# krisbrud/gym-auv

Hardware: AMD Instinct MI355X
Metric: env-steps/sec (higher is better)
Workload: dtype f64; 1 GPU; 4096 envs x 180 sensors per GPU, 50 static polygon obstacles (BASELINE configs[2]); envs_per_gpu=4096, n_sensors=180, total_envs=4096, parallelism=env-shard x1 (no step-path collective), ranks=1, hipgraph_steps=0, steps_per_launch=64, sub_batches=1, api=multi, step_mode=one_launch, roofline_step_mode=one_launch, actions=uniform, worlds_per_env=2, collective_backend=none, episodes_finished=212

## Files before the change

### gym_auv_amd/csrc/k1_dynamics.hip

```cpp
#include <hip/hip_ext.h>

#include "auv_device.h"

namespace {

struct Vec6 {
  double v[6];
};

#define AUV_DIVC(x, c) auv_div_const((x), (c), 1.0 / (c))
__device__ __forceinline__ double auv_div_const(double x, double c, double rc) {
  const double q = x * rc;
  const double r = fma(-q, c, x);
  return fma(r, rc, q);
}

struct Heading0 {
  double psi, s, c;
};

__device__ __forceinline__ Heading0 heading0(double psi) {
  Heading0 h;
  h.psi = psi;
  sincos(auv_princip(psi), &h.s, &h.c);
  return h;
}

__device__ __forceinline__ void stage_sincos(const Heading0& h0, const double psi, double* s, double* c) {
  const double dl = psi - h0.psi;
  if (fabs(dl) <= 0.125) {
    const double z = dl * dl;
    double ps = fma(z, 1.0 / 6227020800.0, -1.0 / 39916800.0);
    ps = fma(z, ps, 1.0 / 362880.0), ps = fma(z, ps, -1.0 / 5040.0), ps = fma(z, ps, 1.0 / 120.0);
    ps = fma(z, ps, -1.0 / 6.0);
    const double sd = fma(dl * z, ps, dl);
    double pc = fma(z, -1.0 / 87178291200.0, 1.0 / 479001600.0);
    pc = fma(z, pc, -1.0 / 3628800.0), pc = fma(z, pc, 1.0 / 40320.0), pc = fma(z, pc, -1.0 / 720.0);
    pc = fma(z, pc, 1.0 / 24.0), pc = fma(z, pc, -0.5);
    const double cd = fma(z, pc, 1.0);
    *s = fma(h0.s, cd, h0.c * sd);
    *c = fma(h0.c, cd, -(h0.s * sd));
  } else {
    sincos(auv_princip(psi), s, c);
  }
}

__device__ __forceinline__ Vec6 state_dot(const Vec6& y, double tau_u, double tau_r, const Heading0& h0) {
  const double m = 23.8, x_g = 0.046, I_z = 1.760, X_udot = -2.0, Y_vdot = -10.0, Y_rdot = 0.0,
               N_rdot = -1.0, N_vdot = 0.0, X_u = -2.0, Y_v = -7.0, Y_r = -0.1, N_v = -0.1, N_r = -0.5;
  const double m11 = m - X_udot, m22 = m - Y_vdot, m23 = m * x_g - Y_rdot, m32 = m * x_g - N_vdot,
               m33 = I_z - N_rdot;
  const double det = m22 * m33 - m23 * m32;
  const double i11 = 1.0 / m11, i22 = m33 / det, i23 = -m23 / det, i32 = -m32 / det, i33 = m22 / det;
  double s, c;
  stage_sincos(h0, y.v[2], &s, &c);
  double u = y.v[3], v = y.v[4], r = y.v[5];
  Vec6 o;
  o.v[0] = c * u + -s * v;
  o.v[1] = s * u + c * v;
  o.v[2] = r;
  double d0 = 2.0 * u;
  double d1 = 7.0 * v + -2.5425 * r;
  double d2 = -2.5425 * v + 1.422 * r;
  double n0 = -X_u * u;
  double n1 = -Y_v * v + (m * u - Y_r) * r;
  double n2 = -N_v * v + (m * x_g * u - N_r) * r;
  double r0 = tau_u - d0 - n0, r1 = 0.0 - d1 - n1, r2 = tau_r - d2 - n2;
  o.v[3] = i11 * r0;
  o.v[4] = i22 * r1 + i23 * r2;
  o.v[5] = i32 * r1 + i33 * r2;
  return o;
}

__device__ __forceinline__ void k1_action(const AuvDev& d, const void* __restrict__ actions, const int e, double* a0, double* a1, const int slot = -1) {
  size_t i = 2 * (size_t)e;
  if (slot >= 0) i += (size_t)slot * 2 * (size_t)d.n;
  else if (d.ring_slots > 1)
    i += (size_t)(d.ring_slot_host >= 0 ? d.ring_slot_host : *d.ring_pos) * 2 * (size_t)d.n;
  if (d.act_f64) {
    const double2 a = *(const double2*)((const double*)actions + i);
    *a0 = a.x, *a1 = a.y;
  } else {
    const float2 a = *(const float2*)((const float*)actions + i);
    *a0 = (double)a.x, *a1 = (double)a.y;
  }
}

__device__ __forceinline__ EnvPre k1_env(const AuvDev& d, const int e, const void* __restrict__ actions, const bool store) {
  const size_t n = (size_t)d.n;
  double a0, a1;
  k1_action(d, actions, e, &a0, &a1);
  if (isnan(a0) || isnan(a1)) a0 = a1 = 0.0;
  const double tu = auv_clip(a0, 0.0, 1.0) * d.cfg.thrust_max;
  const double tr = auv_clip(a1, -1.0, 1.0) * d.cfg.moment_max;
  const double h = d.cfg.dt;
  Vec6 y, t;
#pragma unroll
  for (int i = 0; i < 6; i++) y.v[i] = d.state[i * n + e];

  const Heading0 h0 = heading0(y.v[2]);
  Vec6 s1 = state_dot(y, tu, tr, h0);
#pragma unroll
  for (int i = 0; i < 6; i++) t.v[i] = y.v[i] + h * s1.v[i] / 4.0;
  Vec6 s2 = state_dot(t, tu, tr, h0);
#pragma unroll
  for (int i = 0; i < 6; i++) t.v[i] = y.v[i] + 3.0 * h * s1.v[i] / 32.0 + 9.0 * h * s2.v[i] / 32.0;
  Vec6 s3 = state_dot(t, tu, tr, h0);
#pragma unroll
  for (int i = 0; i < 6; i++)
    t.v[i] = y.v[i] + AUV_DIVC(1932.0 * h * s1.v[i], 2197.0) - AUV_DIVC(7200.0 * h * s2.v[i], 2197.0) +
             AUV_DIVC(7296.0 * h * s3.v[i], 2197.0);
  Vec6 s4 = state_dot(t, tu, tr, h0);
#pragma unroll
  for (int i = 0; i < 6; i++)
    t.v[i] = y.v[i] + AUV_DIVC(439.0 * h * s1.v[i], 216.0) - 8.0 * h * s2.v[i] + AUV_DIVC(3680.0 * h * s3.v[i], 513.0) -
             AUV_DIVC(845.0 * h * s4.v[i], 4104.0);
  Vec6 s5 = state_dot(t, tu, tr, h0);
#pragma unroll
  for (int i = 0; i < 6; i++)
    t.v[i] = y.v[i] - AUV_DIVC(8.0 * h * s1.v[i], 27.0) + 2 * h * s2.v[i] - AUV_DIVC(3544.0 * h * s3.v[i], 2565.0) +
             AUV_DIVC(1859.0 * h * s4.v[i], 4104.0) - AUV_DIVC(11.0 * h * s5.v[i], 40.0);
  Vec6 s6 = state_dot(t, tu, tr, h0);
#pragma unroll
  for (int i = 0; i < 6; i++)
    t.v[i] = y.v[i] + h * (AUV_DIVC(16.0 * s1.v[i], 135.0) + AUV_DIVC(6656.0 * s3.v[i], 12825.0) +
                           AUV_DIVC(28561.0 * s4.v[i], 56430.0) - AUV_DIVC(9.0 * s5.v[i], 50.0) + AUV_DIVC(2.0 * s6.v[i], 55.0));
  t.v[2] = auv_princip(t.v[2]);
  EnvPre pre;
  pre.cnt = d.counters[e];
  pre.cnt.y += 1;
#pragma unroll
  for (int i = 0; i < 6; i++) pre.s[i] = t.v[i];
  if (store) {
#pragma unroll
    for (int i = 0; i < 6; i++) d.state[i * n + e] = t.v[i];
    d.counters[e].y = pre.cnt.y;
  }
  return pre;
}

#define K1_GROUP 8
template <int K> __device__ __forceinline__ int k1_group_bcast32(const int x) {
  static_assert(K >= 0 && K < 8, "lane of the group");
  constexpr int q = K % 4, qp = q | (q << 2) | (q << 4) | (q << 6);
  const int a = __builtin_amdgcn_update_dpp(0, x, qp, 0xF, 0xF, true);
  return K < 4 ? __builtin_amdgcn_update_dpp(a, a, 0x114, 0xF, 0xA, false) : __builtin_amdgcn_update_dpp(a, a, 0x104, 0xF, 0x5, false);
}
template <int K> __device__ __forceinline__ double k1_group_bcast(const double t) {
  return __hiloint2double(k1_group_bcast32<K>(__double2hiint(t)), k1_group_bcast32<K>(__double2loint(t)));
}
__device__ __forceinline__ double k1_group(const AuvDev& d, const void* __restrict__ actions, const int e, const int lane,
                                           const double* y_in = nullptr, const int slot = -1, const double2* a_in = nullptr) {
  const int c = lane % K1_GROUP, gbase = lane - c;
  const size_t n = (size_t)d.n;
  const bool own = c < 6;
  double a0, a1;
  if (a_in) a0 = a_in->x, a1 = a_in->y;
  else k1_action(d, actions, e, &a0, &a1, slot);
  if (isnan(a0) || isnan(a1)) a0 = a1 = 0.0;
  const double tu = auv_clip(a0, 0.0, 1.0) * d.cfg.thrust_max;
  const double tr = auv_clip(a1, -1.0, 1.0) * d.cfg.moment_max;
  const double h = d.cfg.dt;
  const double y = y_in ? *y_in : d.state[(size_t)(own ? c : 0) * n + e];
  (void)gbase;
  const Heading0 h0 = heading0(k1_group_bcast<2>(y));
  auto sdot = [&](double t) {
    Vec6 v;
    v.v[0] = 0.0, v.v[1] = 0.0;
    v.v[2] = k1_group_bcast<2>(t), v.v[3] = k1_group_bcast<3>(t);
    v.v[4] = k1_group_bcast<4>(t), v.v[5] = k1_group_bcast<5>(t);
    const Vec6 o = state_dot(v, tu, tr, h0);
    double r = o.v[0];
#pragma unroll
    for (int i = 1; i < 6; i++) r = (c == i) ? o.v[i] : r;
    return r;
  };
  const double s1 = sdot(y);
  double t = y + h * s1 / 4.0;
  const double s2 = sdot(t);
  t = y + 3.0 * h * s1 / 32.0 + 9.0 * h * s2 / 32.0;
  const double s3 = sdot(t);
  t = y + AUV_DIVC(1932.0 * h * s1, 2197.0) - AUV_DIVC(7200.0 * h * s2, 2197.0) + AUV_DIVC(7296.0 * h * s3, 2197.0);
  const double s4 = sdot(t);
  t = y + AUV_DIVC(439.0 * h * s1, 216.0) - 8.0 * h * s2 + AUV_DIVC(3680.0 * h * s3, 513.0) - AUV_DIVC(845.0 * h * s4, 4104.0);
  const double s5 = sdot(t);
  t = y - AUV_DIVC(8.0 * h * s1, 27.0) + 2 * h * s2 - AUV_DIVC(3544.0 * h * s3, 2565.0) + AUV_DIVC(1859.0 * h * s4, 4104.0) -
      AUV_DIVC(11.0 * h * s5, 40.0);
  const double s6 = sdot(t);
  t = y + h * (AUV_DIVC(16.0 * s1, 135.0) + AUV_DIVC(6656.0 * s3, 12825.0) + AUV_DIVC(28561.0 * s4, 56430.0) -
               AUV_DIVC(9.0 * s5, 50.0) + AUV_DIVC(2.0 * s6, 55.0));
  if (c == 2) t = auv_princip(t);
  return t;
}

#ifndef AUV_DEVICE_FUNCS_ONLY
__global__ void __launch_bounds__(AUV_BLOCK) k1_dynamics(AuvDev d, const void* __restrict__ actions) {
  const int tid = blockIdx.x * blockDim.x + threadIdx.x;
  const int lane = threadIdx.x % AUV_WAVE;
  const int c = lane % K1_GROUP;
  const size_t n = (size_t)d.n;
  const bool live = tid / K1_GROUP < d.ne;
  const int e = d.e0 + (live ? tid / K1_GROUP : d.ne - 1);
  const double t = k1_group(d, actions, e, lane);
  if (live && c < 6) d.state[(size_t)c * n + e] = t;
  if (live && c == 0) d.counters[e].y += 1;
}
#endif

}

#ifndef AUV_DEVICE_FUNCS_ONLY
void auv_launch_k1(const AuvDev& d0, const void* actions, int dtype, hipStream_t st, hipEvent_t ev0, hipEvent_t ev1) {
  AuvDev d = d0;
  d.act_f64 = dtype == AUV_F64;
  const int per_block = AUV_BLOCK / K1_GROUP;
  dim3 grid((d.ne + per_block - 1) / per_block), block(AUV_BLOCK);
  hipExtLaunchKernelGGL(k1_dynamics, grid, block, 0, st, ev0, ev1, 0, d, actions);
}
#endif
```

### gym_auv_amd/csrc/k2_lidar.hip

```cpp
#include "auv_device.h"

namespace {

#define K2_KIND_MASK 0xff
#define K2_PIP_FLAG 0x100
struct ObsLds {
  int kind;
  int seg_off;
  int nseg;
  int start;
  int count;
  int wind;
};

struct EnvHdr {
  double px, py;
  double cpsi, spsi;
  int n_act;
  int pad[3];
};

__device__ __forceinline__ unsigned long long d2u(double x) { return (unsigned long long)__double_as_longlong(x); }
__device__ __forceinline__ double u2d(unsigned long long x) { return __longlong_as_double((long long)x); }

__device__ __forceinline__ int wrap_ray(int i, int S) {
  if (i < 0) i += S;
  if (i < 0) i += S;
  if (i >= S) i -= S;
  return i;
}

struct MoverSegs {
  double c, s, x, y, wd;
  __device__ __forceinline__ void vertex(int k, double& vx, double& vy) const {
    const double bx = (k <= 1) ? -wd / 2 : (k == 3 ? 3.0 / 2 * wd : wd / 2);
    const double by = (k == 0 || k == 4) ? -wd / 2 : (k == 3 ? 0.0 : wd / 2);
    const double x0 = 5.0 * wd / 18.0;
    const double xo = x0 - x0 * c, yo = 0.0 - x0 * s;
    vx = (c * bx + -s * by + xo) + x;
    vy = (s * bx + c * by + yo) + y;
  }
  __device__ __forceinline__ double4 operator[](int i) const {
    double ax, ay, bx, by;
    vertex(i, ax, ay);
    vertex(i == 4 ? 0 : i + 1, bx, by);
    return make_double4(ax, ay, bx, by);
  }
};

#ifndef K2_SEG_CAP
#define K2_SEG_CAP 96
#endif
#define K2_SEG_CAP_MIN 32
#ifndef K2_HIT_S
#define K2_HIT_S 256
#endif
#ifndef K2_RAW_CAP
#define K2_RAW_CAP 192
#endif
#ifndef K2_ITEM_RAYS
#define K2_ITEM_RAYS 6
#endif

__host__ __device__ __forceinline__ size_t k2_slice_bytes(int S, int k_max, int m_max, int cap) {
  size_t b = sizeof(EnvHdr) + (size_t)m_max * 32 + (size_t)cap * 32 + (size_t)S * 16 + (size_t)m_max * 16 +
             (size_t)S * 8 + (size_t)m_max * 8 + (size_t)k_max * sizeof(ObsLds) + (size_t)cap * 4 +
             (size_t)k_max * 4 + (size_t)(k_max + 1) * 4 + (size_t)k_max * 4 + (size_t)cap * 2 +
             (size_t)(cap + 2) * 2;
  return (b + 15) & ~(size_t)15;
}
__host__ __device__ __forceinline__ size_t k2_slice_bytes(const AuvDev& d) { return k2_slice_bytes(d.cfg.n_sensors, d.k_max, d.m_max, d.seg_cap); }

struct Slice {
  EnvHdr* hdr;
  double4* mvrot;
  double4* stage;
  double2* rayv;
  double2* mvcull;
  unsigned long long* dbits;
  double* mvw;
  ObsLds* obs;
  short2* span;
  int* act;
  int* sbase;
  int* par;
  unsigned short* owner;
  unsigned short* ioff;
  int cap;
  int* hits;
  double* hitw;
};

__device__ __forceinline__ MoverSegs mover_segs(const double4 rot, const double wd) {
  MoverSegs ms;
  ms.c = rot.x, ms.s = rot.y, ms.x = rot.z, ms.y = rot.w, ms.wd = wd;
  return ms;
}

__device__ __forceinline__ Slice carve(unsigned char* p, int S, int k_max, int m_max, int cap) {
  Slice s;
  s.hdr = (EnvHdr*)p;
  s.mvrot = (double4*)(s.hdr + 1);
  s.stage = s.mvrot + m_max;
  s.rayv = (double2*)(s.stage + cap);
  s.mvcull = s.rayv + S;
  s.dbits = (unsigned long long*)(s.mvcull + m_max);
  s.mvw = (double*)(s.dbits + S);
  s.obs = (ObsLds*)(s.mvw + m_max);
  s.span = (short2*)(s.obs + k_max);
  s.act = (int*)(s.span + cap);
  s.sbase = s.act + k_max;
  s.par = s.sbase + k_max + 1;
  s.owner = (unsigned short*)(s.par + k_max);
  s.ioff = s.owner + cap;
  s.cap = cap;
  const size_t r1 = 32 * (size_t)(m_max + cap), r2 = (size_t)((unsigned char*)(s.ioff + cap + 2) - (unsigned char*)s.mvw);
  const size_t hb = ((size_t)4 * S + 7) & ~(size_t)7;
  s.hits = nullptr, s.hitw = nullptr;
  if (S <= K2_HIT_S && hb + (size_t)8 * S <= r1) s.hits = (int*)s.mvrot, s.hitw = (double*)((unsigned char*)s.mvrot + hb);
  else if (S <= K2_HIT_S && hb <= r1 && (size_t)8 * S <= r2) s.hits = (int*)s.mvrot, s.hitw = s.mvw;
  return s;
}
__device__ __forceinline__ Slice carve(unsigned char* p, const AuvDev& d) { return carve(p, d.cfg.n_sensors, d.k_max, d.m_max, d.seg_cap); }

__device__ __forceinline__ void test_pair(const double4 w, const double tn, const double2 r,
                                          unsigned long long* slot) {
  const double den = r.x * w.w - r.y * w.z;
  const double un = w.x * r.y - w.y * r.x;
  const bool neg = den < 0.0;
  const double dn = neg ? -den : den, t1 = neg ? -tn : tn, u1 = neg ? -un : un;
  const bool hit = (dn != 0.0) & (t1 >= 0.0) & (t1 <= dn) & (u1 >= 0.0) & (u1 <= dn);
  if (hit) atomicMin(slot, d2u(tn / den));
}

__device__ __forceinline__ void test_pair_signed(const double4 ws, const double ta, const double2 r, unsigned long long* slot) {
  const double dn = r.x * ws.w - r.y * ws.z;
  const double u1 = ws.x * r.y - ws.y * r.x;
  const bool hit = (dn > 0.0) & (ta <= dn) & (u1 >= 0.0) & (u1 <= dn);
  if (hit) atomicMin(slot, d2u(ta / dn));
}

template <typename SegPtr>
__device__ __forceinline__ void sweep_unstaged(const ObsLds& o, int tid, int nthr, int S, double px, double py,
                                               const double2* rayv, unsigned long long* dbits, SegPtr g) {
  const int total = o.count * o.nseg;
  for (int q = tid; q < total; q += nthr) {
    const int ro = q / o.nseg, si = q - ro * o.nseg;
    const int i = wrap_ray(o.start + ro, S);
    const double4 s = g[si];
    const double4 w = make_double4(s.x - px, s.y - py, s.z - s.x, s.w - s.y);
    test_pair(w, w.x * w.w - w.y * w.z, rayv[i], &dbits[i]);
  }
}

template <typename SegPtr>
__device__ __forceinline__ int inside_flag_wave(double px, double py, SegPtr g, int nseg, int lane) {
  int on_any = 0, cross = 0;
  for (int sb = 0; sb < nseg; sb += AUV_WAVE) {
    const int si = sb + lane;
    bool on = false, cr = false;
    if (si < nseg) {
      const double4 s = g[si];
      const double sx = s.z - s.x, sy = s.w - s.y, dxa = px - s.x, dya = py - s.y;
      const double len2 = sx * sx + sy * sy, dot = dxa * sx + dya * sy;
      if (len2 == 0.0 || dot <= 0.0) on = (dxa == 0.0 && dya == 0.0);
      else if (dot >= len2) on = (px == s.z && py == s.w);
      else on = ((s.y - py) * sx - (s.x - px) * sy) == 0.0;
      if ((s.y > py) != (s.w > py)) cr = px < s.x + (py - s.y) * (s.z - s.x) / (s.w - s.y);
    }
    on_any |= __any(on);
    cross += __popcll(__ballot(cr));
  }
  return (on_any ? 2 : 0) | (cross & 1);
}

__device__ __forceinline__ void k2_stage_beams(const AuvDev& d, const int lane, const Slice& L) {
  const int S = d.cfg.n_sensors;
  for (int i = lane; i < S; i += AUV_WAVE) L.rayv[i] = d.beam_cs[i];
}

__device__ __forceinline__ void k2_rays(const AuvDev& d, const int lane, const Slice& L, const bool staged = false) {
  const int S = d.cfg.n_sensors;
  const double R = d.cfg.sensor_range;
  const double px = L.hdr->px, py = L.hdr->py;
  double sin_psi, cos_psi;
  if (S <= 4 * AUV_WAVE) {
    double2 b[4];
    if (!staged) {
#pragma unroll
      for (int q = 0; q < 4; q++) {
        const int i = q * AUV_WAVE + lane;
        b[q] = d.beam_cs[i < S ? i : 0];
      }
    }
    cos_psi = L.hdr->cpsi, sin_psi = L.hdr->spsi;
#pragma unroll
    for (int q = 0; q < 4; q++) {
      if (q * AUV_WAVE >= S) break;
      const int i = q * AUV_WAVE + lane;
      if (i < S) {
        if (staged) b[q] = L.rayv[i];
        const double c = cos_psi * b[q].x - sin_psi * b[q].y, s = sin_psi * b[q].x + cos_psi * b[q].y;
        double ex = px + c * R, ey = py + s * R;
        L.rayv[i] = make_double2(ex - px, ey - py);
        L.dbits[i] = d2u(2.0);
      }
    }
  } else {
    cos_psi = L.hdr->cpsi, sin_psi = L.hdr->spsi;
    for (int i = lane; i < S; i += AUV_WAVE) {
      const double2 b = staged ? L.rayv[i] : d.beam_cs[i];
      const double c = cos_psi * b.x - sin_psi * b.y, s = sin_psi * b.x + cos_psi * b.y;
      double ex = px + c * R, ey = py + s * R;
      L.rayv[i] = make_double2(ex - px, ey - py);
      L.dbits[i] = d2u(2.0);
    }
  }
  auv_wave_lds_sync();
}

template <bool WT = false, bool LD = false>
__device__ __forceinline__ void k2_movers(const AuvDev& d, const int e, const int lane, const Slice& L, const EnvDesc& ed,
                                          const int advance_movers) {
  const long long m0 = ed.m0;
  const int M = ed.M;
  for (int m = lane; m < M; m += AUV_WAVE) {
    double4 st = auv_ld4<LD>(&d.mover[(size_t)e * d.m_max + m]);
    const double4 par_m = d.mv_param[m0 + m];
    if (advance_movers) {
      const double dt = d.cfg.dt;
      const long long voff = d.mv_vtab_off[m0 + m];
      const int vlen = d.mv_vtab_len[m0 + m];
      st.w += dt;
      int idx = (int)floor(st.w);
      if (idx >= (int)par_m.w - 1) {
        st.w = 0.0;
        idx = 0;
        st.x = par_m.y;
        st.y = par_m.z;
      }
      if (idx > vlen - 1) idx = vlen - 1;
      double2 v = d.mv_vtab[voff + idx];
      double dx = dt * v.x, dy = dt * v.y;
      st.z = atan2(dy, dx);
      st.x = st.x + dx;
      st.y = st.y + dy;
      auv_st<WT>(&d.mover[(size_t)e * d.m_max + m], st);
    }
    const double wd = par_m.x;
    double s, c;
    sincos(st.z, &s, &c);
    const double x0 = 5.0 * wd / 18.0, dxc = wd / 2.0 - x0;
    L.mvcull[m] = make_double2(st.x + x0 + c * dxc, st.y + s * dxc);
    if (fabs(c) < 2.5e-16) c = 0.0;
    if (fabs(s) < 2.5e-16) s = 0.0;
    L.mvrot[m] = make_double4(c, s, st.x, st.y);
    L.mvw[m] = wd;
  }
}

struct K2Pre {
  int4 meta;
  double cx, cy, rho;
  uint8_t near;
};
template <bool LD = false>
__device__ __forceinline__ K2Pre k2_prefetch(const AuvDev& d, const int e, const int lane, const EnvDesc& ed) {
  K2Pre p;
  p.meta = make_int4(0, 0, 0, 0), p.cx = p.cy = p.rho = 0.0, p.near = 0;
  if (lane < ed.K) {
    p.meta = d.obs_meta[ed.k0 + lane];
    p.cx = d.obs_cull[3 * (ed.k0 + lane)], p.cy = d.obs_cull[3 * (ed.k0 + lane) + 1], p.rho = d.obs_cull[3 * (ed.k0 + lane) + 2];
    p.near = auv_ld<LD>(&d.nearby[(size_t)e * d.k_max + lane]);
  }
  return p;
}

template <bool WT = false>
__device__ __forceinline__ int k2_front(const AuvDev& d, const int e, const int lane, const Slice& L, const int advance_movers,
                        const EnvPre* pre = nullptr, const int movers_done = 0,
                        const K2Pre* kp = nullptr, const bool beams_staged = false, int2* lim_defer = nullptr) {
  const int S = d.cfg.n_sensors;
  const size_t n = (size_t)d.n;
  const int4 cnt = pre ? pre->cnt : d.counters[e];
  const double px = pre ? pre->s[0] : d.state[0 * n + e], py = pre ? pre->s[1] : d.state[1 * n + e],
               psi = pre ? pre->s[2] : d.state[2 * n + e];
  const EnvDesc ed = (pre && pre->ed) ? *pre->ed : d.env_desc[e];
  {
    double sn, co;
    sincos(psi, &sn, &co);
    if (lane == 0) L.hdr->cpsi = co, L.hdr->spsi = sn;
  }
  const long long k0 = ed.k0;
  const int K = ed.K;
  const double R = d.cfg.sensor_range, W = d.cfg.vessel_width;
  const double dangle = d.derived[4], inv_dangle = d.derived[5];
  if (lane == 0) {
    L.hdr->px = px, L.hdr->py = py;
    L.hdr->n_act = 0;
  }

  if (!movers_done) k2_movers<WT>(d, e, lane, L, ed, advance_movers);
  if (!d.cfg.use_lidar) return 0;

  const bool refresh = (cnt.y % d.cfg.sensor_interval_load_obstacles) == 0;
  if (refresh) {
    for (int kb = 0; kb < K; kb += AUV_WAVE) {
      const int k = kb + lane;
      int4 meta = make_int4(0, 0, 0, 0);
      double dc = 0.0, rho = 0.0;
      int state = 0;
      if (k < K) {
        meta = d.obs_meta[k0 + k];
        double cx, cy;
        if (meta.x == AUV_OBS_MOVER) {
          const double2 c2 = L.mvcull[meta.w];
          cx = c2.x, cy = c2.y, rho = L.mvw[meta.w] * sqrt(5.0) / 2.0;
        } else {
          cx = d.obs_cull[3 * (k0 + k)], cy = d.obs_cull[3 * (k0 + k) + 1], rho = d.obs_cull[3 * (k0 + k) + 2];
        }
        dc = sqrt((px - cx) * (px - cx) + (py - cy) * (py - cy));
        state = (dc - rho - W >= R + 1e-9) ? 0 : ((dc + rho - W < R - 1e-9) ? 1 : 2);
      }
      unsigned long long pin = __ballot(state == 2 && meta.x != AUV_OBS_RING && dc <= rho * (1.0 + 1e-9) + 1e-9);
      while (pin) {
        const int src = __ffsll((long long)pin) - 1;
        pin &= pin - 1;
        const int kind = __shfl(meta.x, src, AUV_WAVE), soff = __shfl(meta.y, src, AUV_WAVE),
                  nseg = __shfl(meta.z, src, AUV_WAVE), mi = __shfl(meta.w, src, AUV_WAVE);
        const int in = (kind == AUV_OBS_MOVER) ? inside_flag_wave(px, py, mover_segs(L.mvrot[mi], L.mvw[mi]), nseg, lane)
                                               : inside_flag_wave(px, py, d.seg + soff, nseg, lane);
// ... 704 lines not shown
```

### gym_auv_amd/csrc/k_step_fused.hip

```cpp
#include <cstdlib>
#include <hip/hip_ext.h>

#define AUV_DEVICE_FUNCS_ONLY
#include "auv_multi_geom.h"
#include "k1_dynamics.hip"
#include "k2_lidar.hip"
#include "k3_nav_reward.hip"

#ifndef AUV_K23_MIN_WAVES
#define AUV_K23_MIN_WAVES 4
#endif

#ifdef AUV_TEST_HOOKS
#define AUV_HOOK_SKEW(d) ((d).pair_skew)
#define AUV_HOOK_FAULT(d) ((d).pair_fault)
#else
#define AUV_HOOK_SKEW(d) 0
#define AUV_HOOK_FAULT(d) 0
#endif

namespace {

#define PAIR_EMPTY AUV_PAIR_EMPTY
#define PAIR_COLLISION AUV_PAIR_COLLISION
// ... 248 lines not shown
    __hip_atomic_store(pair_word + e, PAIR_EMPTY, __ATOMIC_RELAXED, __HIP_MEMORY_SCOPE_AGENT);
    __hip_atomic_store(k1_pkt + 8 * (size_t)e + 7, 0ull, __ATOMIC_RELAXED, __HIP_MEMORY_SCOPE_AGENT);
    __hip_atomic_store(hd + 7, 0ull, __ATOMIC_RELAXED, __HIP_MEMORY_SCOPE_AGENT);
    RewardIn in;
    const int collision = word == PAIR_COLLISION;
    in.closeness_reward = collision ? 0.0 : __longlong_as_double((long long)word);
    in.path_reward = no.rew_path, in.reached = no.reached, in.goal = no.goal, in.progress = no.progress;
    in.u = no.u, in.v = no.v, in.yaw_rate = no.r;
    in.cum = cum_in;
    in.cte100 = no.cte100, in.cte_sum = cte_sum_in;
    st.info64[8 * (size_t)e] = collision;
    do_reset = reward_apply(st, e, collision, cnt, in, reward_out, done_out, false);
  }
  unsigned long long m = __ballot(do_reset);
  if (m) {
    while (m) {
      const int src = __ffsll((long long)m) - 1;
      m &= m - 1;
      const int er2 = auv_uniform(__shfl(e, src, AUV_WAVE));
      const int wr = auv_uniform(__shfl(w, src, AUV_WAVE)), ep = auv_uniform(__shfl(cnt.z, src, AUV_WAVE));
      const AuvDev* dp = dk.self;
      asm volatile("" : "+s"(dp));
      const AuvDev& dr = *(const AuvDev*)(const __attribute__((address_space(4))) AuvDev*)dp;
      restore_env(dr, er2, auv_next_world_wave(dr, wr, lane), lane, ep, obs_out);
    }
  }
#ifdef AUV_STAMPS
  if (live && c == 0) d.stamps[(size_t)e * 16 + 15] = wall_clock64();
#endif
}

__global__ void __launch_bounds__(AUV_WAVE, AUV_K23_MIN_WAVES) k_step_roles(AuvDev dk, const void* __restrict__ actions,
                                                                           float* __restrict__ obs_out,
                                                                           float* __restrict__ reward_out,
                                                                           uint8_t* __restrict__ done_out) {
  const AuvDev& d = dk;
  extern __shared__ __align__(16) unsigned char smem[];
  const int lane = threadIdx.x;
  const int ne = d.ne;
  const int nk = 8 * ((ne + 63) / 64);
  const int nb = 8 * ((ne + 7) / 8);
  const int b = (int)blockIdx.x;
  if (b < nk) {
    __builtin_amdgcn_s_setprio(3);
    const int g = lane / K1_GROUP, c = lane % K1_GROUP;
    const int er = 8 * (8 * (b / 8) + g) + (b % 8);
    const bool live = er < ne;
    const int eg = d.e0 + (live ? er : ne - 1);
    const int y = d.counters[eg].y + 1;
    const int aborted = auv_uniform(*d.abort_flag);
    double t = 0.0;
    if (!aborted) t = k1_group(d, actions, eg, lane);
    unsigned long long* pk = d.k1_pkt + 8 * (size_t)eg;
    const unsigned long long word = aborted ? (c == 6 ? (unsigned long long)ROLES_ABORT_COUNTER : 0ull)
                                            : (c < 6 ? (unsigned long long)__double_as_longlong(t) : (c == 6 ? (unsigned long long)(unsigned)y : 0ull));
    const unsigned long long mark = roles_mark(roles_group_xor(word));
    if (live && !(AUV_HOOK_FAULT(d) == 2 && eg == d.e0))
      __hip_atomic_store(pk + c, c < 7 ? word : mark, __ATOMIC_RELAXED, __HIP_MEMORY_SCOPE_AGENT);
    if (d.ring_slots > 1 && d.ring_slot_host == -1 && lane == 0) {
      const int old = __hip_atomic_fetch_add(d.k1_done, 1, __ATOMIC_RELAXED, __HIP_MEMORY_SCOPE_AGENT);
      if (old == nk - 1) {
        *d.ring_pos = (*d.ring_pos + 1) % d.ring_slots;
        __hip_atomic_store(d.k1_done, 0, __ATOMIC_RELAXED, __HIP_MEMORY_SCOPE_AGENT);
      }
    }
#ifdef AUV_STAMPS
    if (live && c == 0) d.stamps[(size_t)eg * 16 + 0] = wall_clock64();
#endif
    return;
  }
  EnvPre pre;
  EnvDesc ed;
  if (b < nk + nb) {
    if (b - nk >= ne) return;
    const int e = auv_uniform(d.e0 + b - nk);
#ifdef AUV_STAMPS
    if (lane == 0) d.stamps[(size_t)e * 16 + 3] = wall_clock64();
#endif
    if (auv_uniform(*d.abort_flag)) return;
    ed = d.env_desc[e];
    pre.cnt = d.counters[e];
    pre.ed = &ed;
    const Slice L = carve(smem, d);
    k2_movers<true>(d, e, lane, L, ed, 1);
    const K2Pre kp = k2_prefetch(d, e, lane, ed);
    k2_stage_beams(d, lane, L);
#ifdef AUV_STAMPS
    if (lane == 0) d.stamps[(size_t)e * 16 + 1] = wall_clock64();
#endif
    {
      const int ws = roles_wait_state(d, e, lane, pre);
      if (ws) {
        if (ws == 2 && ed.M > 0 && lane == 0) auv_st<true>(d.broken + e, (uint8_t)1);
        return;
      }
    }
#ifdef AUV_STAMPS
    if (lane == 0) d.stamps[(size_t)e * 16 + 2] = wall_clock64();
#endif
    int n_act = 0;
    int2 lim0 = make_int2(INT32_MIN, INT32_MIN);
    if (AUV_RUN_L(d, 1)) n_act = k2_front<true>(d, e, lane, L, 1, &pre, 1, &kp, true, &lim0);
#ifdef AUV_STAMPS
    if (lane == 0) d.stamps[(size_t)e * 16 + 8] = wall_clock64();
#endif
    if (AUV_RUN_L(d, 3)) k2_stage_and_pairs(d, L, lane, n_act, pre.s[2]);
#ifdef AUV_STAMPS
    if (lane == 0) d.stamps[(size_t)e * 16 + 11] = wall_clock64();
#endif
    double term = 0.0;
    const int collision = k2_back<true>(d, e, lane, L, n_act, obs_out, &term, &lim0);
#ifdef AUV_STAMPS
    if (lane == 0) d.stamps[(size_t)e * 16 + 4] = wall_clock64();
#endif
    pair_publish_lidar(d, e, lane, collision, term);
#ifdef AUV_STAMPS
    if (lane == 0) d.stamps[(size_t)e * 16 + 14] = wall_clock64();
#endif
  } else if (b < nk + 2 * nb + AUV_HOOK_SKEW(d)) {
    const int el = b - nk - nb - AUV_HOOK_SKEW(d);
    if (el < 0 || el >= ne) return;
    const int e = auv_uniform(d.e0 + el);
    ed = d.env_desc[e];
    pre.cnt = d.counters[e];
    pre.ed = &ed;
#ifdef AUV_STAMPS
    if (lane == 0) d.stamps[(size_t)e * 16 + 12] = wall_clock64();
#endif
    if (roles_wait_state(d, e, lane, pre)) return;
#ifdef AUV_STAMPS
    if (lane == 0) d.stamps[(size_t)e * 16 + 5] = wall_clock64();
#endif
    NavNear nr;
    nr.A = nr.B = make_double2(0.0, 0.0), nr.cum = 0.0;
    if (AUV_RUN_N(d, 1)) {
      int* list = (int*)smem;
      const NavSpec sp = nav_bounds(d, e, lane, list, pre.s[0], pre.s[1], &ed);
      if (AUV_RUN_N(d, 2)) nr = nav_nearest(d, e, lane, list, pre.s[0], pre.s[1], sp);
    }
    roles_publish_search(d, e, lane, nr);
#ifdef AUV_STAMPS
    if (lane == 0) d.stamps[(size_t)e * 16 + 6] = wall_clock64();
#endif
  } else {
    const int f = b - nk - 2 * nb - AUV_HOOK_SKEW(d);
    if (f < 0 || f >= nk) return;
    __builtin_amdgcn_s_setprio(2);
    roles_finish_wave(d, f, lane, obs_out, reward_out, done_out);
  }
}

#define CARRY_WORDS 24

#ifdef AUV_STAMPS_MULTI
#define MSTAMP(e, k) do { if (lane == 0) stamp[(size_t)(e) * 16 + (k)] = wall_clock64(); } while (0)
#define MSTAMP_IF(cond, e, k) do { if (cond) stamp[(size_t)(e) * 16 + (k)] = wall_clock64(); } while (0)
#define MSTAMP_PARAM , unsigned long long* stamp
#define MSTAMP_ARG , stamp
#else
#define MSTAMP(e, k) do { } while (0)
#define MSTAMP_IF(cond, e, k) do { } while (0)
#define MSTAMP_PARAM
#define MSTAMP_ARG
#endif

__device__ __forceinline__ unsigned long long carry_ed_word(const EnvDesc& ed, const int i) {
  switch (i) {
    case 0: return (unsigned long long)ed.k0;
    case 1: return (unsigned long long)ed.m0;
    case 2: return (unsigned long long)ed.p0;
    case 3: return (unsigned long long)ed.c0;
    case 4: return (unsigned long long)ed.kn0;
    case 5: return (unsigned long long)(unsigned)ed.K | ((unsigned long long)(unsigned)ed.M << 32);
    case 6: return (unsigned long long)(unsigned)ed.P | ((unsigned long long)(unsigned)ed.nch << 32);
    default: return (unsigned long long)(unsigned)ed.nk | ((unsigned long long)(unsigned)ed.w << 32);
  }
}
__device__ __forceinline__ void carry_ed_from(EnvDesc& ed, const unsigned long long w[8]) {
  ed.k0 = (long long)w[0], ed.m0 = (long long)w[1], ed.p0 = (long long)w[2], ed.c0 = (long long)w[3], ed.kn0 = (long long)w[4];
  ed.K = (int)(unsigned)w[5], ed.M = (int)(unsigned)(w[5] >> 32), ed.P = (int)(unsigned)w[6], ed.nch = (int)(unsigned)(w[6] >> 32);
  ed.nk = (int)(unsigned)w[7], ed.w = (int)(unsigned)(w[7] >> 32);
}

__device__ __forceinline__ int carry_wait_wave(const AuvDev& d, const int e, const int lane, const unsigned long long tagmix, EnvDesc& ed, int4& cnt) {
  const unsigned long long* cw = d.carry + CARRY_WORDS * (size_t)e;
  unsigned long long v = 0ull;
  for (int polls = 0;; polls++) {
    if (lane < CARRY_WORDS) v = __hip_atomic_load(cw + lane, __ATOMIC_RELAXED, __HIP_MEMORY_SCOPE_AGENT);
    const unsigned long long ma = roles_lane_word(v, 7), mb = roles_lane_word(v, 20);
    if (ma != 0ull && mb != 0ull) {
      unsigned long long xa = roles_lane_word(v, 0), xb = roles_lane_word(v, 8);
#pragma unroll
      for (int i = 1; i < 7; i++) xa ^= roles_lane_word(v, i);
#pragma unroll
      for (int i = 9; i < 20; i++) xb ^= roles_lane_word(v, i);
      if (roles_mark(xa ^ tagmix) == ma && roles_mark(xb ^ tagmix) == mb) break;
    }
    if ((polls & 31) == 31 && auv_uniform(__hip_atomic_load(d.abort_flag, __ATOMIC_RELAXED, __HIP_MEMORY_SCOPE_AGENT))) return 2;
    if (polls == (AUV_HOOK_FAULT(d) ? (1 << 12) : PAIR_POLL_LIMIT)) {
      if (lane == 0) auv_st<true>(d.broken + e, (uint8_t)1);
      roles_give_up(d, d.e0, d.ne, 6, lane);
      return 1;
    }
    __builtin_amdgcn_s_sleep(ROLES_POLL_SLEEP);
  }
  unsigned long long w[8];
#pragma unroll
  for (int i = 0; i < 8; i++) w[i] = roles_lane_word(v, 12 + i);
  carry_ed_from(ed, w);
  const unsigned long long c6 = roles_lane_word(v, 6), c8 = roles_lane_word(v, 8);
  cnt = make_int4((int)(unsigned)c6, (int)(unsigned)(c6 >> 32), (int)(unsigned)c8, 0);
  return 0;
}

template <bool MULTI>
__device__ __forceinline__ void roles_finish_wave_multi(const AuvDev& dk, const int f, const int lane, float* __restrict__ obs_out,
                                                        float* __restrict__ reward_out, uint8_t* __restrict__ done_out, const int step,
                                                        const bool last_step, const unsigned long long tagmix, const unsigned long long tagmix_prev MSTAMP_PARAM) {
  const __attribute__((address_space(4))) AuvDev* dc = (const __attribute__((address_space(4))) AuvDev*)dk.self;
  const AuvDev& d = *(const AuvDev*)dc;
  StepTabs st;
  st.cfg.min_cumulative_reward = dc->cfg.min_cumulative_reward, st.cfg.min_goal_distance = dc->cfg.min_goal_distance;
  st.cfg.min_path_progress = dc->cfg.min_path_progress, st.cfg.look_ahead_distance = dc->cfg.look_ahead_distance;
  st.cfg.max_timesteps = dc->cfg.max_timesteps, st.cfg.rewarder = dc->cfg.rewarder, st.cfg.test_mode = dc->cfg.test_mode;
  st.cfg.auto_reset = dc->cfg.auto_reset, st.cfg.n_sensors = dc->cfg.n_sensors, st.cfg.use_lidar = dc->cfg.use_lidar;
  st.cfg.obs_channels = dc->cfg.obs_channels, st.pool_ns = dc->pool_ns;
  st.knot_s = dc->knot_s, st.knot_coef = dc->knot_coef;
  st.info64 = dc->info64, st.nav64 = dc->nav64, st.obs64 = dc->obs64, st.rew_path = dc->rew_path, st.reward64 = dc->reward64;
  st.step_info = dc->step_info, st.episode = dc->episode, st.ep_log = dc->ep_log, st.ep_log_count = dc->ep_log_count;
  st.ep_log_cap = dc->ep_log_cap, st.world_idx = dc->world_idx, st.counters = dc->counters;
  st.fw_serial = nullptr, st.n = dc->n;
  st.ring_slots = 1, st.ring_slot_host = 0, st.ring_pos = nullptr;
  unsigned long long* const pair_word = dc->pair_word;
  unsigned long long* const k1_pkt = dc->k1_pkt;
  unsigned long long* const nav_hand = dc->nav_hand;
  unsigned long long* const carry = dc->carry;
  const EnvDesc* const env_desc = dc->env_desc;
  const double* const world_scalar = dc->world_scalar;
  double* const state = dc->state;
  uint8_t* const broken = dc->broken;
  const int n_envs = dc->n;
  const int ne = dk.ne, e0 = dk.e0;
  const int g = lane / K1_GROUP, c = lane % K1_GROUP;
  const int er = 8 * (8 * (f / 8) + g) + (f % 8);
  const bool live = er < ne;
  const int e = e0 + (live ? er : ne - 1);
  const int limit = AUV_HOOK_FAULT(dk) ? (1 << 12) : PAIR_POLL_LIMIT;
  int4 cnt;
  double cum_in, cte_sum_in, maxp_in;
  EnvDesc ed;
  unsigned long long* const cw = carry + CARRY_WORDS * (size_t)e;
  if (step == 0) {
    cnt = st.counters[e];
    cum_in = st.info64[8 * (size_t)e + 4], cte_sum_in = st.info64[8 * (size_t)e + 7], maxp_in = st.info64[8 * (size_t)e + 5];
    ed = env_desc[e];
  } else {
    unsigned long long v0 = 0ull, v1 = 0ull, v2 = 0ull;
    bool ok = !live;
    for (int polls = 0;; polls++) {
      if (!ok) {
        v0 = __hip_atomic_load(cw + c, __ATOMIC_RELAXED, __HIP_MEMORY_SCOPE_AGENT);
        v1 = __hip_atomic_load(cw + 8 + c, __ATOMIC_RELAXED, __HIP_MEMORY_SCOPE_AGENT);
        v2 = __hip_atomic_load(cw + 16 + c, __ATOMIC_RELAXED, __HIP_MEMORY_SCOPE_AGENT);
      }
      const unsigned long long xb = roles_group_xor(v1) ^ roles_group_xor(c < 4 ? v2 : 0ull), mb = roles_group_word(v2, 4);
      ok = !live || (roles_record_ok(v0, c, tagmix_prev) && mb != 0ull && roles_mark(xb ^ tagmix_prev) == mb);
      if (!__any(!ok)) break;
      if ((polls & 31) == 31 && auv_uniform(__hip_atomic_load(dc->abort_flag, __ATOMIC_RELAXED, __HIP_MEMORY_SCOPE_AGENT))) return;
      if (polls == limit) {
        if (live && c == 0) auv_st<true>(broken + e, (uint8_t)1);
        roles_give_up(d, e0, ne, 6, lane);
        return;
      }
      __builtin_amdgcn_s_sleep(ROLES_POLL_SLEEP);
    }
    const unsigned long long c6 = roles_group_word(v0, 6), c8 = roles_group_word(v1, 0);
    cnt = make_int4((int)(unsigned)c6, (int)(unsigned)(c6 >> 32), (int)(unsigned)c8, 0);
    cum_in = roles_group_value(v1, 1), maxp_in = roles_group_value(v1, 2), cte_sum_in = roles_group_value(v1, 3);
    unsigned long long w[8];
#pragma unroll
    for (int i = 0; i < 4; i++) w[i] = roles_group_word(v1, 4 + i);
#pragma unroll
    for (int i = 0; i < 4; i++) w[4 + i] = roles_group_word(v2, i);
    carry_ed_from(ed, w);
    if (!live) ed = env_desc[e];
  }
  const int w = ed.w;
  TailIn t;
  t.kn0 = ed.kn0, t.nk = ed.nk;
  {
    const double* ws = world_scalar + 8 * (size_t)ed.w;
    t.L = ws[0], t.goal_x = ws[1], t.goal_y = ws[2];
    t.knot_first = st.knot_s[ed.kn0], t.knot_last = st.knot_s[ed.kn0 + ed.nk - 1];
    t.maxp_in = maxp_in;
  }
  const unsigned long long* pk = k1_pkt + 8 * (size_t)e;
  unsigned long long* hd = nav_hand + 8 * (size_t)e;
  unsigned long long vp = 0ull, vh = 0ull;
  bool okp = !live, okh = !live, aborted = false;
  for (int polls = 0;; polls++) {
    if (!okp) vp = __hip_atomic_load(pk + c, __ATOMIC_RELAXED, __HIP_MEMORY_SCOPE_AGENT);
    if (!okh) vh = __hip_atomic_load(hd + c, __ATOMIC_RELAXED, __HIP_MEMORY_SCOPE_AGENT);
    okp = !live || roles_record_ok(vp, c, tagmix);
    aborted = live && okp && (unsigned)roles_group_word(vp, 6) == ROLES_ABORT_COUNTER;
    okh = !live || aborted || roles_record_ok(vh, c, tagmix);
    if (!__any(!(okp && okh))) break;
    if (polls == limit) {
      if (live && c == 0) auv_st<true>(broken + e, (uint8_t)1);
      roles_give_up(d, e0, ne, 3, lane);
      return;
    }
    __builtin_amdgcn_s_sleep(ROLES_POLL_SLEEP);
  }
  if (__any(aborted)) return;
  t.px = roles_group_value(vp, 0), t.py = roles_group_value(vp, 1), t.psi = roles_group_value(vp, 2);
  t.u = roles_group_value(vp, 3), t.v = roles_group_value(vp, 4), t.r = roles_group_value(vp, 5);
  cnt.y = (int)(unsigned)roles_group_word(vp, 6);
  t.nr.A = make_double2(roles_group_value(vh, 0), roles_group_value(vh, 1));
  t.nr.B = make_double2(roles_group_value(vh, 2), roles_group_value(vh, 3));
  t.nr.cum = roles_group_value(vh, 4);
  NavOut no;
  no.rew_path = no.reached = no.goal = no.progress = no.u = no.v = no.r = no.cte100 = no.maxp = 0.0;
  unsigned long long word = live ? __hip_atomic_load(pair_word + e, __ATOMIC_RELAXED, __HIP_MEMORY_SCOPE_AGENT) : 0ull;
  no = nav_tail<K1_GROUP>(st, e, c, live, t, obs_out);
  if (live && c < 6) state[(size_t)c * (size_t)n_envs + e] = __longlong_as_double((long long)vp);
  for (int polls = 0;; polls++) {
    if (!__any(word == PAIR_EMPTY)) break;
    if (word == PAIR_EMPTY) word = __hip_atomic_load(pair_word + e, __ATOMIC_RELAXED, __HIP_MEMORY_SCOPE_AGENT);
    if (!__any(word == PAIR_EMPTY)) break;
    if (polls == limit) {
      if (live && c == 0) auv_st<true>(broken + e, (uint8_t)1);
      roles_give_up(d, e0, ne, 1, lane);
      return;
    }
    __builtin_amdgcn_s_sleep(ROLES_POLL_SLEEP);
  }
  MSTAMP_IF(live && c == 0, e, 14);
  int do_reset = 0;
  double co[2] = {0.0, 0.0};
  if (live && c == 0) {
    __hip_atomic_store(pair_word + e, PAIR_EMPTY, __ATOMIC_RELAXED, __HIP_MEMORY_SCOPE_AGENT);
// ... 282 lines not shown
```

### gym_auv_amd/csrc/k_step_multi_body.inc

```
  extern __shared__ __align__(16) unsigned char smem[];
#ifdef AUV_STAMPS_MULTI
  const unsigned long long t_entry = wall_clock64();
#endif
  const int lane = threadIdx.x;
  const int ne = d.ne;
  const bool cohorts = lead_dyn >= 0;
  const AuvMultiWave wa = auv_multi_decode_steps(blockIdx.x, ne, n_steps);
  const AuvMultiWave wc = auv_multi_decode_cohorts(blockIdx.x, ne, n_steps, lead_dyn, lag_fin, magic_c);
  const int step = auv_uniform(cohorts ? wc.step : wa.step);
  const int role = auv_uniform(cohorts ? wc.role : wa.role), bi = auv_uniform(cohorts ? wc.bi : wa.bi);
  if (step >= n_steps) return;
#if STEP_MULTI_REC
  {
    obs_out += (unsigned long long)(unsigned)step * obs_stride;
    reward_out += (unsigned long long)(unsigned)step * reward_stride;
    done_out += (unsigned long long)(unsigned)step * done_stride;
  }
#endif
  const unsigned long long tagmix = roles_tagmix(seq0 + (unsigned long long)step + 1ull), tagmix_prev = roles_tagmix(seq0 + (unsigned long long)step);
#ifdef AUV_STAMPS_MULTI
  unsigned long long* const stamp = d.stamps + (step == n_steps / 2 ? (size_t)0 : (size_t)16 * (size_t)d.n);
#endif
  if (role == 0) {
    __builtin_amdgcn_s_setprio(3);
    const int b = bi;
    const int g = lane / K1_GROUP, c = lane % K1_GROUP;
    const int er = 8 * (8 * (b / 8) + g) + (b % 8);
    const bool live = er < ne;
    const int eg = d.e0 + (live ? er : ne - 1);
    int y, gave_up = 0;
    double y0 = 0.0;
    MSTAMP_IF(live && c == 0, eg, 10);
    const int ab_early = __hip_atomic_load(d.abort_flag, __ATOMIC_RELAXED, __HIP_MEMORY_SCOPE_AGENT);
    double act0, act1;
    k1_action(d, actions, eg, &act0, &act1, (first_slot + step) % n_slots);
    if (step == 0) {
      y = d.counters[eg].y + 1;
    } else {
      const unsigned long long* cw = d.carry + CARRY_WORDS * (size_t)eg;
      unsigned long long v = 0ull;
      bool ok = !live;
      for (int polls = 0;; polls++) {
        if (!ok) v = __hip_atomic_load(cw + c, __ATOMIC_RELAXED, __HIP_MEMORY_SCOPE_AGENT);
        ok = !live || roles_record_ok(v, c, tagmix_prev);
        if (!__any(!ok)) break;
        if ((polls & 31) == 31 && auv_uniform(__hip_atomic_load(d.abort_flag, __ATOMIC_RELAXED, __HIP_MEMORY_SCOPE_AGENT))) {
          gave_up = 1;
          break;
        }
        if (polls == (AUV_HOOK_FAULT(d) ? (1 << 12) : PAIR_POLL_LIMIT)) {
          if (live && c == 0) auv_st<true>(d.broken + eg, (uint8_t)1);
          roles_give_up(d, d.e0, d.ne, 6, lane);
          gave_up = 1;
          break;
        }
        __builtin_amdgcn_s_sleep(ROLES_POLL_SLEEP);
      }
      y0 = __longlong_as_double((long long)v);
      y = (int)(unsigned)(roles_group_word(v, 6) >> 32) + 1;
    }
    const int aborted = gave_up | auv_uniform(ab_early);
    double t = 0.0;
    MSTAMP_IF(live && c == 0, eg, 11);
    const double2 act = make_double2(act0, act1);
    if (!aborted) t = k1_group(d, actions, eg, lane, step == 0 ? nullptr : &y0, (first_slot + step) % n_slots, &act);
    unsigned long long* pk = d.k1_pkt + 8 * (size_t)eg;
    const unsigned long long word = aborted ? (c == 6 ? (unsigned long long)ROLES_ABORT_COUNTER : 0ull)
                                            : (c < 6 ? (unsigned long long)__double_as_longlong(t) : (c == 6 ? (unsigned long long)(unsigned)y : 0ull));
    const unsigned long long mark = roles_mark(roles_group_xor(word) ^ tagmix);
    if (live && !(AUV_HOOK_FAULT(d) == 2 && eg == d.e0 && step == 0))
      __hip_atomic_store(pk + c, c < 7 ? word : mark, __ATOMIC_RELAXED, __HIP_MEMORY_SCOPE_AGENT);
    MSTAMP_IF(live && c == 0, eg, 12);
    return;
  }
  EnvPre pre;
  EnvDesc ed;
  if (role == 1) {
    const int e = auv_uniform(d.e0 + bi);
    MSTAMP(e, 0);
    const int ab_early = __hip_atomic_load(d.abort_flag, __ATOMIC_RELAXED, __HIP_MEMORY_SCOPE_AGENT);
    const unsigned long long pk_first = __hip_atomic_load(d.k1_pkt + 8 * (size_t)e + (lane & 7), __ATOMIC_RELAXED, __HIP_MEMORY_SCOPE_AGENT);
    const Slice L = carve(smem, d);
    K2Pre kp;
    if (step == 0) {
      ed = d.env_desc[e];
      pre.cnt = d.counters[e];
      pre.ed = &ed;
      if (auv_uniform(ab_early)) return;
      k2_movers<true>(d, e, lane, L, ed, 1);
      kp = k2_prefetch(d, e, lane, ed);
    } else {
      if (carry_wait_wave(d, e, lane, tagmix_prev, ed, pre.cnt)) return;
      if (auv_uniform(ab_early)) return;
      pre.ed = &ed;
      k2_movers<true, true>(d, e, lane, L, ed, 1);
      kp = k2_prefetch<true>(d, e, lane, ed);
    }
    k2_stage_beams(d, lane, L);
    {
      const int ws = roles_wait_state(d, e, lane, pre, tagmix, true, pk_first);
      if (ws) {
        if (ws == 2 && ed.M > 0 && lane == 0) auv_st<true>(d.broken + e, (uint8_t)1);
        return;
      }
    }
    MSTAMP(e, 2);
    int2 lim0 = make_int2(INT32_MIN, INT32_MIN);
    const int n_act = k2_front<true>(d, e, lane, L, 1, &pre, 1, &kp, true, &lim0);
    k2_stage_and_pairs(d, L, lane, n_act, pre.s[2]);
    MSTAMP(e, 4);
    double term = 0.0;
    const int collision = k2_back<true>(d, e, lane, L, n_act, obs_out, &term, &lim0);
    pair_publish_lidar(d, e, lane, collision, term);
    MSTAMP(e, 5);
#ifdef AUV_STAMPS_MULTI
    if (lane == 0) stamp[(size_t)e * 16 + 1] = t_entry;
    __builtin_amdgcn_s_waitcnt(0x0F70);
    MSTAMP(e, 3);
#endif
  } else if (role == 2) {
    const int e = auv_uniform(d.e0 + bi);
    MSTAMP(e, 6);
    const unsigned long long pk_first = __hip_atomic_load(d.k1_pkt + 8 * (size_t)e + (lane & 7), __ATOMIC_RELAXED, __HIP_MEMORY_SCOPE_AGENT);
    if (step == 0) {
      ed = d.env_desc[e];
      pre.cnt = d.counters[e];
    } else if (carry_wait_wave(d, e, lane, tagmix_prev, ed, pre.cnt)) {
      return;
    }
#ifdef AUV_STAMPS_MULTI
    if (lane == 0) stamp[(size_t)e * 16 + 7] = t_entry;
#endif
    pre.ed = &ed;
    if (roles_wait_state(d, e, lane, pre, tagmix, true, pk_first)) return;
    MSTAMP(e, 8);
    NavNear nr;
    int* list = (int*)smem;
    const NavSpec sp = nav_bounds(d, e, lane, list, pre.s[0], pre.s[1], &ed);
    nr = nav_nearest(d, e, lane, list, pre.s[0], pre.s[1], sp);
    roles_publish_search(d, e, lane, nr, tagmix);
    MSTAMP(e, 9);
  } else {
    const int f = bi;
    __builtin_amdgcn_s_setprio(2);
#ifdef AUV_STAMPS_MULTI
    const int fer = 8 * (8 * (f / 8) + lane / K1_GROUP) + (f % 8);
    const bool fst = fer < ne && lane % K1_GROUP == 0;
#endif
    MSTAMP_IF(fst, d.e0 + fer, 13);
    roles_finish_wave_multi<true>(d, f, lane, obs_out, reward_out, done_out, step, step == n_steps - 1, tagmix, tagmix_prev MSTAMP_ARG);
    MSTAMP_IF(fst, d.e0 + fer, 15);
  }
```

Measured before the change: 186.2 million env-steps/s.

## Issue carry load early and stage beam table via async global-to-LDS loads

In the lidar role wave, the first carry-word poll is now issued together with the abort and packet loads at entry, and its value is passed into the wait loop. Beam direction staging moves to direct global_load_lds transfers issued before the movers and prefetch work instead of a register round-trip afterwards. Hit-buffer carving is deferred until just before the back half, and k1_group takes the state by value instead of through a pointer. The aim is to overlap global-memory latency with other setup work on the wave's critical path. In exchange it adds an explicit vmcnt(0) wait at entry and relies on address-space casts and on implicit ordering of the LDS writes before the beams are read.

```diff
diff --git a/gym_auv_amd/csrc/k1_dynamics.hip b/gym_auv_amd/csrc/k1_dynamics.hip
--- a/gym_auv_amd/csrc/k1_dynamics.hip
+++ b/gym_auv_amd/csrc/k1_dynamics.hip
@@ -150,7 +150,8 @@
   return __hiloint2double(k1_group_bcast32<K>(__double2hiint(t)), k1_group_bcast32<K>(__double2loint(t)));
 }
 __device__ __forceinline__ double k1_group(const AuvDev& d, const void* __restrict__ actions, const int e, const int lane,
-                                           const double* y_in = nullptr, const int slot = -1, const double2* a_in = nullptr) {
+                                           const bool have_y = false, const double y_val = 0.0, const int slot = -1,
+                                           const double2* a_in = nullptr) {
   const int c = lane % K1_GROUP, gbase = lane - c;
   const size_t n = (size_t)d.n;
   const bool own = c < 6;
@@ -161,7 +162,7 @@
   const double tu = auv_clip(a0, 0.0, 1.0) * d.cfg.thrust_max;
   const double tr = auv_clip(a1, -1.0, 1.0) * d.cfg.moment_max;
   const double h = d.cfg.dt;
-  const double y = y_in ? *y_in : d.state[(size_t)(own ? c : 0) * n + e];
+  const double y = have_y ? y_val : d.state[(size_t)(own ? c : 0) * n + e];
   (void)gbase;
   const Heading0 h0 = heading0(k1_group_bcast<2>(y));
   auto sdot = [&](double t) {
diff --git a/gym_auv_amd/csrc/k2_lidar.hip b/gym_auv_amd/csrc/k2_lidar.hip
--- a/gym_auv_amd/csrc/k2_lidar.hip
+++ b/gym_auv_amd/csrc/k2_lidar.hip
@@ -97,7 +97,7 @@
   return ms;
 }
 
-__device__ __forceinline__ Slice carve(unsigned char* p, int S, int k_max, int m_max, int cap) {
+__device__ __forceinline__ Slice carve_base(unsigned char* p, int S, int k_max, int m_max, int cap) {
   Slice s;
   s.hdr = (EnvHdr*)p;
   s.mvrot = (double4*)(s.hdr + 1);
@@ -114,11 +114,19 @@
   s.owner = (unsigned short*)(s.par + k_max);
   s.ioff = s.owner + cap;
   s.cap = cap;
+  s.hits = nullptr, s.hitw = nullptr;
+  return s;
+}
+__device__ __forceinline__ void carve_hits(Slice& s, int S, int m_max, int cap) {
   const size_t r1 = 32 * (size_t)(m_max + cap), r2 = (size_t)((unsigned char*)(s.ioff + cap + 2) - (unsigned char*)s.mvw);
   const size_t hb = ((size_t)4 * S + 7) & ~(size_t)7;
   s.hits = nullptr, s.hitw = nullptr;
   if (S <= K2_HIT_S && hb + (size_t)8 * S <= r1) s.hits = (int*)s.mvrot, s.hitw = (double*)((unsigned char*)s.mvrot + hb);
   else if (S <= K2_HIT_S && hb <= r1 && (size_t)8 * S <= r2) s.hits = (int*)s.mvrot, s.hitw = s.mvw;
+}
+__device__ __forceinline__ Slice carve(unsigned char* p, int S, int k_max, int m_max, int cap) {
+  Slice s = carve_base(p, S, k_max, m_max, cap);
+  carve_hits(s, S, m_max, cap);
   return s;
 }
 __device__ __forceinline__ Slice carve(unsigned char* p, const AuvDev& d) { return carve(p, d.cfg.n_sensors, d.k_max, d.m_max, d.seg_cap); }
@@ -177,6 +185,19 @@
 __device__ __forceinline__ void k2_stage_beams(const AuvDev& d, const int lane, const Slice& L) {
   const int S = d.cfg.n_sensors;
   for (int i = lane; i < S; i += AUV_WAVE) L.rayv[i] = d.beam_cs[i];
+}
+
+__device__ __forceinline__ void k2_stage_beams_direct(const AuvDev& d, const int lane, const Slice& L) {
+  const AuvDev* dp = &d;
+  asm volatile("" : "+s"(dp));
+  const __attribute__((address_space(4))) AuvDev* dc = (const __attribute__((address_space(4))) AuvDev*)dp;
+  const int S = dc->cfg.n_sensors;
+  const double2* src = dc->beam_cs + lane;
+  typedef __attribute__((address_space(1))) const void* gptr_t;
+  typedef __attribute__((address_space(3))) void* lptr_t;
+#pragma nounroll
+  for (int q = 0; q < S; q += AUV_WAVE)
+    if (q + lane < S) __builtin_amdgcn_global_load_lds((gptr_t)(src + q), (lptr_t)(L.rayv + q), 16, 0, 0);
 }
 
 __device__ __forceinline__ void k2_rays(const AuvDev& d, const int lane, const Slice& L, const bool staged = false) {
diff --git a/gym_auv_amd/csrc/k_step_fused.hip b/gym_auv_amd/csrc/k_step_fused.hip
--- a/gym_auv_amd/csrc/k_step_fused.hip
+++ b/gym_auv_amd/csrc/k_step_fused.hip
@@ -424,6 +424,7 @@
 
 #define CARRY_WORDS 24
 
+#define AUV_WAITCNT_VMCNT0 0x0F70
 #ifdef AUV_STAMPS_MULTI
 #define MSTAMP(e, k) do { if (lane == 0) stamp[(size_t)(e) * 16 + (k)] = wall_clock64(); } while (0)
 #define MSTAMP_IF(cond, e, k) do { if (cond) stamp[(size_t)(e) * 16 + (k)] = wall_clock64(); } while (0)
@@ -454,11 +455,16 @@
   ed.nk = (int)(unsigned)w[7], ed.w = (int)(unsigned)(w[7] >> 32);
 }
 
-__device__ __forceinline__ int carry_wait_wave(const AuvDev& d, const int e, const int lane, const unsigned long long tagmix, EnvDesc& ed, int4& cnt) {
+__device__ __forceinline__ unsigned long long carry_request(const AuvDev& d, const int e, const int lane) {
+  return lane < CARRY_WORDS ? __hip_atomic_load(d.carry + CARRY_WORDS * (size_t)e + lane, __ATOMIC_RELAXED, __HIP_MEMORY_SCOPE_AGENT) : 0ull;
+}
+__device__ __forceinline__ int carry_wait_wave(const AuvDev& d, const int e, const int lane, const unsigned long long tagmix, EnvDesc& ed, int4& cnt,
+                                               const bool have_first = false, const unsigned long long v_first = 0ull) {
   const unsigned long long* cw = d.carry + CARRY_WORDS * (size_t)e;
   unsigned long long v = 0ull;
   for (int polls = 0;; polls++) {
-    if (lane < CARRY_WORDS) v = __hip_atomic_load(cw + lane, __ATOMIC_RELAXED, __HIP_MEMORY_SCOPE_AGENT);
+    if (have_first && polls == 0) v = v_first;
+    else if (lane < CARRY_WORDS) v = __hip_atomic_load(cw + lane, __ATOMIC_RELAXED, __HIP_MEMORY_SCOPE_AGENT);
     const unsigned long long ma = roles_lane_word(v, 7), mb = roles_lane_word(v, 20);
     if (ma != 0ull && mb != 0ull) {
       unsigned long long xa = roles_lane_word(v, 0), xb = roles_lane_word(v, 8);
diff --git a/gym_auv_amd/csrc/k_step_multi_body.inc b/gym_auv_amd/csrc/k_step_multi_body.inc
--- a/gym_auv_amd/csrc/k_step_multi_body.inc
+++ b/gym_auv_amd/csrc/k_step_multi_body.inc
@@ -63,7 +63,7 @@
     double t = 0.0;
     MSTAMP_IF(live && c == 0, eg, 11);
     const double2 act = make_double2(act0, act1);
-    if (!aborted) t = k1_group(d, actions, eg, lane, step == 0 ? nullptr : &y0, (first_slot + step) % n_slots, &act);
+    if (!aborted) t = k1_group(d, actions, eg, lane, step != 0, y0, (first_slot + step) % n_slots, &act);
     unsigned long long* pk = d.k1_pkt + 8 * (size_t)eg;
     const unsigned long long word = aborted ? (c == 6 ? (unsigned long long)ROLES_ABORT_COUNTER : 0ull)
                                             : (c < 6 ? (unsigned long long)__double_as_longlong(t) : (c == 6 ? (unsigned long long)(unsigned)y : 0ull));
@@ -78,9 +78,12 @@
   if (role == 1) {
     const int e = auv_uniform(d.e0 + bi);
     MSTAMP(e, 0);
+    __builtin_amdgcn_s_waitcnt(AUV_WAITCNT_VMCNT0);
     const int ab_early = __hip_atomic_load(d.abort_flag, __ATOMIC_RELAXED, __HIP_MEMORY_SCOPE_AGENT);
     const unsigned long long pk_first = __hip_atomic_load(d.k1_pkt + 8 * (size_t)e + (lane & 7), __ATOMIC_RELAXED, __HIP_MEMORY_SCOPE_AGENT);
-    const Slice L = carve(smem, d);
+    const unsigned long long cw_first = carry_request(d, e, lane);
+    Slice L = carve_base(smem, d.cfg.n_sensors, d.k_max, d.m_max, d.seg_cap);
+    k2_stage_beams_direct(d, lane, L);
     K2Pre kp;
     if (step == 0) {
       ed = d.env_desc[e];
@@ -90,13 +93,12 @@
       k2_movers<true>(d, e, lane, L, ed, 1);
       kp = k2_prefetch(d, e, lane, ed);
     } else {
-      if (carry_wait_wave(d, e, lane, tagmix_prev, ed, pre.cnt)) return;
+      if (carry_wait_wave(d, e, lane, tagmix_prev, ed, pre.cnt, true, cw_first)) return;
       if (auv_uniform(ab_early)) return;
       pre.ed = &ed;
       k2_movers<true, true>(d, e, lane, L, ed, 1);
       kp = k2_prefetch<true>(d, e, lane, ed);
     }
-    k2_stage_beams(d, lane, L);
     {
       const int ws = roles_wait_state(d, e, lane, pre, tagmix, true, pk_first);
       if (ws) {
@@ -110,12 +112,18 @@
     k2_stage_and_pairs(d, L, lane, n_act, pre.s[2]);
     MSTAMP(e, 4);
     double term = 0.0;
+    {
+      const AuvDev* dp = &d;
+      asm volatile("" : "+s"(dp));
+      const __attribute__((address_space(4))) AuvDev* dc = (const __attribute__((address_space(4))) AuvDev*)dp;
+      carve_hits(L, dc->cfg.n_sensors, dc->m_max, dc->seg_cap);
+    }
     const int collision = k2_back<true>(d, e, lane, L, n_act, obs_out, &term, &lim0);
     pair_publish_lidar(d, e, lane, collision, term);
     MSTAMP(e, 5);
 #ifdef AUV_STAMPS_MULTI
     if (lane == 0) stamp[(size_t)e * 16 + 1] = t_entry;
-    __builtin_amdgcn_s_waitcnt(0x0F70);
+    __builtin_amdgcn_s_waitcnt(AUV_WAITCNT_VMCNT0);
     MSTAMP(e, 3);
 #endif
   } else if (role == 2) {
```

Result: faster. 194.6 million env-steps/s, median of 6 (+4.5%).
